# ClimateImpactLab/climate_toolbox

Hardware: AMD Instinct MI355X
Metric: gridcell-region-timesteps/sec (higher is better)
Workload: dtype f32

## Files before the change

climate_toolbox_amd/csrc/wagg_dense.hip:

```cpp
#include <algorithm>
#include <cfloat>
#include <chrono>
#include <cmath>
#include <limits>
#include <cstdlib>
#include <type_traits>

#include "wagg_dense_int.h"
#include "wagg_entry.h"

namespace wagg {

constexpr int D_MT = 23;
constexpr int D_BN = 256;
constexpr int D_ROWB = 128;
constexpr int D_THREADS = 512;
constexpr int D_WTB = D_BN * D_ROWB;
constexpr int D_WSLOTS = D_WTB / 16;
static_assert(D_WTB / 1024 == 32, "4 one-KiB W pieces per wave");
constexpr int d_xt_bytes(int mt) { return mt * 16 * D_ROWB; }
constexpr int d_buf_bytes(int mt) { return d_xt_bytes(mt) + D_WTB; }
static_assert(2 * d_buf_bytes(D_MT) <= 160 * 1024, "LDS budget");

typedef float f32x4 __attribute__((ext_vector_type(4)));
// ... 621 lines not shown
            dreg = ctx.take_input<int32_t>((size_t)n);
            dw = ctx.take_input<double>((size_t)n);
            if (!(drow || dcell) || !dreg || !dw) { set_error("build arena too small for the table"); return WAGG_ENOMEM; }
            int rc = rowptr ? copy_to_device(drow, rowptr, sizeof(int64_t) * ((size_t)G + 1), true, ctx.st)
                            : copy_to_device(dcell, cell_idx, sizeof(int32_t) * (size_t)n, true, ctx.st);
            if (rc == WAGG_OK) rc = copy_to_device(dreg, region_code, sizeof(int32_t) * (size_t)n, true, ctx.st);
            if (rc == WAGG_OK) rc = copy_to_device(dw, w_eff, sizeof(double) * (size_t)n, true, ctx.st);
            if (rc != WAGG_OK) return rc;
        }
        t_up = wall_s() - t0;
        WAGG_BUILD_STAMP(ctx, "upload");
        if (int rc = build_sorted_entries(ctx, dcell, drow, dreg, dw, n, G, R, kg, &se, general_sort)) return rc;
    }
    uint32_t *bitmap, *word_rank = nullptr;
    WAGG_TAKE(bitmap, ctx, uint32_t, n_words);
    WAGG_HIP(hipMemsetAsync(bitmap, 0, sizeof(uint32_t) * (size_t)n_words, ctx.st));
    const unsigned nblk = (unsigned)((se.n_u + 255) / 256);
    if (se.n_u > 0) {
        hipLaunchKernelGGL((table_tiles_kernel<T>), dim3(nblk), dim3(256), 0, ctx.st, (const uint64_t *)se.key.p, se.n_u, kg, n_kt, bitmap);
        WAGG_HIP(hipGetLastError());
    }
    WAGG_BUILD_STAMP(ctx, "den + tile census");
    std::vector<uint32_t> hbits, hrank;
    std::vector<int64_t> tiles;
    try {
        hbits.resize((size_t)n_words);
        hrank.resize((size_t)n_words);
        WAGG_HIP(staged_d2h(hbits.data(), bitmap, sizeof(uint32_t) * hbits.size(), ctx.st));
        int64_t cnt = 0;
        for (int64_t i = 0; i < n_words; ++i) { hrank[(size_t)i] = (uint32_t)cnt; cnt += __builtin_popcount(hbits[(size_t)i]); }
        tiles.reserve((size_t)cnt);
        for (int64_t i = 0; i < n_words; ++i)
            for (uint32_t m = hbits[(size_t)i]; m; m &= m - 1) tiles.push_back(i * 32 + __builtin_ctz(m));
    } catch (const std::bad_alloc &) { set_error("host allocation failed"); return WAGG_ENOMEM; }
    const double fill_all = (double)se.n_u / ((double)G * (double)R);
    int64_t walked = 0;
    if (se.n_u > 0) { if (int rc = spmm_list_cost(ctx, se, &walked)) return rc; }
    WAGG_BUILD_STAMP(ctx, "bitmap to host + list cost");
    const FormCost cost = table_form_cost(G, (int)sizeof(T), (int64_t)tiles.size(), n_tiles_all, walked, geo.n_rb, n_buckets, n_nt);
    bool tiled, entries;
    pick_table_form(cost, &tiled, &entries);
    if (flags == WAGG_DENSE_FORCE_FULL) { tiled = false; entries = false; }
    else if (flags == WAGG_DENSE_FORCE_TILES) { tiled = true; entries = false; }
    else if (flags == WAGG_DENSE_FORCE_ENTRIES) { tiled = false; entries = true; }
#ifdef WAGG_DIAG
    if (getenv("WAGG_DENSE_NO_TILED") && tiled) { tiled = false; entries = fill_all < SPMM_MAX_FILL; }
#else
    (void)fill_all;
#endif
    int rc = dense_alloc<T>(G, R, out, tiled ? (int64_t)tiles.size() : -1, entries);
    if (rc != WAGG_OK) return rc;
    wagg_dense *d = *out;
    WAGG_BUILD_STAMP(ctx, "plan alloc");
    auto fail = [&](int code) { (void)ctx.sync(); delete d; *out = nullptr; return code; };
    if (entries) {
        ctx.release_to(0);
        rc = spmm_build_from_sorted<T>(ctx, d, se);
        if (rc != WAGG_OK) return fail(rc);
    } else {
        hipError_t e = hipMemsetAsync(d->W.p, 0, 16 * (size_t)d->w_slots(), ctx.st);
        if (e == hipSuccess && tiled) e = dense_set_tiles(d, tiles, nullptr, ctx.st);
        if (e == hipSuccess && tiled) {
            word_rank = ctx.take<uint32_t>((size_t)n_words);
            e = word_rank ? staged_h2d(word_rank, hrank.data(), sizeof(uint32_t) * hrank.size(), ctx.st) : hipErrorOutOfMemory;
        }
        if (e == hipSuccess && se.n_u > 0) {
            hipLaunchKernelGGL((table_scatter_kernel<T>), dim3(nblk), dim3(256), 0, ctx.st, (const uint64_t *)se.key.p, (const double *)se.w.p,
                               se.n_u, kg, n_kt, (const uint32_t *)bitmap, (const uint32_t *)word_rank, reinterpret_cast<T *>(d->W.p));
            e = hipGetLastError();
        }
        if (e != hipSuccess) { set_error("densify: %s", hipGetErrorString(e)); return fail(WAGG_EHIP); }
    }
    hipError_t e = hipMemcpyAsync(d->den64.p, se.den.p, sizeof(double) * (size_t)R, hipMemcpyDeviceToDevice, ctx.st);
    if (e != hipSuccess) { set_error("densify den: %s", hipGetErrorString(e)); return fail(WAGG_EHIP); }
    rc = dense_den_to_host(d, ctx.st);
    if (rc == WAGG_OK) rc = dense_finish_scales(d, ctx.st);
    if (rc != WAGG_OK) return fail(rc);
    e = ctx.sync();
    if (e != hipSuccess) { set_error("plan build: %s", hipGetErrorString(e)); return fail(WAGG_EHIP); }
    WAGG_BUILD_STAMP(ctx, "pack + den to host");
    if (entries) d->sp.nnz = se.n_u;
    d->nnz_table = se.n_u;
    d->est_row_s[0] = cost.t_full; d->est_row_s[1] = cost.t_tiled; d->est_row_s[2] = cost.t_entries;
    d->walked_entries = walked;
    d->one_pass_sort = se.chunkwise;
    d->build.upload_s = t_up;
    d->build.total_s = wall_s() - t0;
    d->build.device_s = d->build.total_s - t_up;
    return WAGG_OK;
}

template <typename T, bool TILED, int MT, bool RM = false>
static const void *mfma_kernel_ptr() {
    if constexpr (TILED) return (const void *)dense_pieces_kernel<T, MT, RM>;
    else return (const void *)dense_mfma_kernel<T, 0, false, MT, RM>;
}
template <typename T>
static const void *pick_full_rm_kernel(int MT, bool rm) {
#define WAGG_PICK(M) case M: return rm ? (const void *)dense_mfma_kernel<T, 0, false, M, true> \
                                       : (const void *)dense_mfma_kernel<T, 256, false, M, false>
    if constexpr (sizeof(T) == 4) {
        switch (MT) { WAGG_PICK(20); WAGG_PICK(21); WAGG_PICK(22); WAGG_PICK(23); default: return nullptr; }
    } else {
        switch (MT) { WAGG_PICK(10); WAGG_PICK(11); default: return nullptr; }
    }
#undef WAGG_PICK
}

template <typename T>
static const void *pick_mfma_kernel(int MT, bool tiled, bool rm = false) {
#define WAGG_PICK(M) case M: return tiled ? (rm ? mfma_kernel_ptr<T, true, M, true>() : mfma_kernel_ptr<T, true, M>()) \
                                          : mfma_kernel_ptr<T, false, M>()
    if constexpr (sizeof(T) == 4) {
        switch (MT) {
            WAGG_PICK(1); WAGG_PICK(2); WAGG_PICK(3); WAGG_PICK(4); WAGG_PICK(5); WAGG_PICK(6); WAGG_PICK(8);
            WAGG_PICK(10); WAGG_PICK(12); WAGG_PICK(14); WAGG_PICK(16); WAGG_PICK(18); WAGG_PICK(20);
            WAGG_PICK(21); WAGG_PICK(22); WAGG_PICK(23);
            default: return nullptr;
        }
    } else {
        switch (MT) {
            WAGG_PICK(1); WAGG_PICK(2); WAGG_PICK(3); WAGG_PICK(4); WAGG_PICK(5); WAGG_PICK(6); WAGG_PICK(8);
            WAGG_PICK(10); WAGG_PICK(11);
            default: return nullptr;
        }
    }
#undef WAGG_PICK
}

static const void *pick_split_kernel(int MT) {
#define WAGG_PICK(M) case M: return (const void *)dense_split_kernel<M>
    switch (MT) {
        WAGG_PICK(1); WAGG_PICK(2); WAGG_PICK(3); WAGG_PICK(4); WAGG_PICK(5); WAGG_PICK(6); WAGG_PICK(8);
        WAGG_PICK(10); WAGG_PICK(12); WAGG_PICK(14); WAGG_PICK(16); WAGG_PICK(18); WAGG_PICK(20);
        WAGG_PICK(21); WAGG_PICK(22); WAGG_PICK(23);
        default: return nullptr;
    }
#undef WAGG_PICK
}

static int dense_apply_split(wagg_dense *d, const float *X_dev, int64_t Tn, int64_t ldx, const PackXfT<float> &xf,
                             float *out_dev, int64_t ldo, int MT, int n_mb, int S, hipStream_t st) {
    const int n_nt = d->n_nt, n_kt = d->n_kt, bm = MT * 16;
    const int kt_per_slice = (n_kt + S - 1) / S;
    const int64_t nblk = (int64_t)n_nt * n_mb * S;
    WAGG_REQUIRE(nblk < (int64_t)0x7fffffff, "grid too large");
    const void *kern = pick_split_kernel(MT);
    if (!kern) { set_error("no split kernel for MT=%d", MT); return WAGG_EINVAL; }
    const size_t need = (size_t)nblk * bm * D_BN;
    if (d->slabs.n < need) WAGG_HIP(d->slabs.alloc(need));
    const int64_t x_slots = (int64_t)n_mb * n_kt * bm * 8;
    if (d->xp.n < (size_t)x_slots * 4) WAGG_HIP(d->xp.alloc((size_t)x_slots * 4));
    if (d->xmax.n < (size_t)Tn) WAGG_HIP(d->xmax.alloc((size_t)Tn));
    const int aligned = ((ldx * sizeof(float)) % 16 == 0) && ((reinterpret_cast<uintptr_t>(X_dev) & 15) == 0) &&
                        (xf.mode != XF_EDD || (reinterpret_cast<uintptr_t>(xf.X2) & 15) == 0);
#ifdef WAGG_DIAG
    if (const char *dbg = MT == D_MT ? getenv("WAGG_SPLIT_DBG") : nullptr) {
        switch (atoi(dbg)) {
            case 1: kern = (const void *)dense_split_kernel<D_MT, 1>; break;
            case 4: kern = (const void *)dense_split_kernel<D_MT, 4>; break;
            case 5: kern = (const void *)dense_split_kernel<D_MT, 5>; break;
            case 8: kern = (const void *)dense_split_kernel<D_MT, 8>; break;
            case 9: kern = (const void *)dense_split_kernel<D_MT, 9>; break;
            default: break;
        }
    }
#endif
    const size_t shmem = 3 * (size_t)d_xt_bytes(MT);
    WAGG_HIP(allow_dynamic_lds(kern, shmem));
    unsigned *xmax = reinterpret_cast<unsigned *>(d->xmax.p);
    WAGG_HIP(hipMemsetAsync(xmax, 0, sizeof(unsigned) * (size_t)Tn, st));
    const int64_t gx = (d->G + 4095) / 4096 < 64 ? (d->G + 4095) / 4096 : 64;
    hipLaunchKernelGGL(dense_rowmax_kernel, dim3((unsigned)gx, (unsigned)Tn), dim3(256), 0, st, X_dev, ldx, d->G, xf, xmax);
    hipLaunchKernelGGL(dense_pack_x_split_kernel, dim3(256 * 16), dim3(256), 0, st, X_dev, Tn, ldx, d->G, n_kt, bm, x_slots, aligned,
                       (const unsigned *)xmax, reinterpret_cast<f16x8 *>(d->xp.p), xf, d->inf_dev);
    WAGG_HIP(hipGetLastError());
    const f16x8 *xp = reinterpret_cast<const f16x8 *>(d->xp.p);
    const float *wp = d->W.p, *wmax = d->wmax.p;
    float *slabs = d->slabs.p;
    int n_kt_a = n_kt, n_nt_a = n_nt, n_mb_a = n_mb, S_a = S, kps = kt_per_slice;
    void *args[] = {&xp, &wp, &wmax, &n_kt_a, &n_nt_a, &n_mb_a, &S_a, &kps, &slabs};
    WAGG_HIP(launch_timed_ptr(true, kern, dim3((unsigned)nblk), dim3(D_THREADS), args, shmem, st));
    hipLaunchKernelGGL(dense_reduce_split_kernel, dim3((unsigned)((d->R + 255) / 256), (unsigned)Tn), dim3(256), 0, st,
                       (const float *)slabs, n_nt, S, bm, d->R, (const float *)d->den32.p, (const unsigned *)xmax, wmax, out_dev, ldo);
    WAGG_HIP(hipGetLastError());
    return WAGG_OK;
}

template <typename T>
static int dense_apply(wagg_dense *d, const T *X_dev, int64_t Tn, int64_t ldx, const PackXfT<T> &xf,
                       T *out_dev, int64_t ldo, int ksplit, void *stream, bool exact = false) {
    typedef typename DT<T>::vec vec_t;
    WAGG_REQUIRE(d != nullptr, "dense plan is NULL");
    WAGG_REQUIRE(d->f64 == (sizeof(T) == 8), "this plan holds %s weights: use the matching wagg_dense_apply_*",
                 d->f64 ? "fp64" : "fp32");
    WAGG_REQUIRE(Tn >= 0, "T < 0");
    if (Tn == 0) return WAGG_OK;
    WAGG_REQUIRE(X_dev && out_dev, "X/out is NULL");
    WAGG_REQUIRE(xf.mode != XF_EDD || xf.X2 != nullptr, "tasmax is NULL");
    WAGG_REQUIRE(ldx >= d->G && ldo >= d->R, "ldx/ldo too small");
    WAGG_REQUIRE(ksplit >= 0 && ksplit % 8 == 0, "ksplit must be 0 or a multiple of 8");
    if (d->spmm) return spmm_apply<T>(d, X_dev, Tn, ldx, xf, out_dev, ldo, (hipStream_t)stream);
    constexpr int64_t ROWS_MAX = (int64_t)(65535 / (DT<T>::MT_MAX * 16)) * (DT<T>::MT_MAX * 16);
    if (Tn > ROWS_MAX) {
        for (int64_t t0 = 0; t0 < Tn; t0 += ROWS_MAX) {
            PackXfT<T> xg = xf;
            if (xg.X2) xg.X2 += t0 * ldx;
            const int64_t rows = Tn - t0 < ROWS_MAX ? Tn - t0 : ROWS_MAX;
            if (int rc = dense_apply<T>(d, X_dev + t0 * ldx, rows, ldx, xg, out_dev + t0 * ldo, ldo, ksplit, stream, exact)) return rc;
        }
        return WAGG_OK;
    }
    const int n_nt = d->n_nt, n_kt = d->n_kt;
    constexpr int BM_MAX = DT<T>::MT_MAX * 16;
    const int n_mb = (int)((Tn + BM_MAX - 1) / BM_MAX);
    const int rows = (int)((Tn + n_mb - 1) / n_mb);
    static const int mts32[] = {1, 2, 3, 4, 5, 6, 8, 10, 12, 14, 16, 18, 20, 21, 22, 23};
    static const int mts64[] = {1, 2, 3, 4, 5, 6, 8, 10, 11};
    int MT = DT<T>::MT_MAX;
    if constexpr (sizeof(T) == 4) { for (int m : mts32) if (m * 16 >= rows) { MT = m; break; } }
    else { for (int m : mts64) if (m * 16 >= rows) { MT = m; break; } }
    const int bm = MT * 16;
    if (n_mb >= 2) {
        const int64_t head = (int64_t)(n_mb - 1) * bm, tail = Tn - head;
        if (tail > 0) {
            int MT_tail = DT<T>::MT_MAX;
            if constexpr (sizeof(T) == 4) { for (int m : mts32) if ((int64_t)m * 16 >= tail) { MT_tail = m; break; } }
            else { for (int m : mts64) if ((int64_t)m * 16 >= tail) { MT_tail = m; break; } }
            if (MT_tail >= 4 && MT - MT_tail >= 2) {
                PackXfT<T> xt = xf;
                if (xt.X2) xt.X2 += head * ldx;
                if (int rc = dense_apply<T>(d, X_dev, head, ldx, xf, out_dev, ldo, ksplit, stream, exact)) return rc;
                return dense_apply<T>(d, X_dev + head * ldx, tail, ldx, xt, out_dev + head * ldo, ldo, ksplit, stream, exact);
            }
        }
    }
    int S = ksplit ? ksplit : pick_ksplit((int64_t)n_nt * n_mb, n_kt);
    if constexpr (sizeof(T) == 4) {
        if (!d->tiled && !exact && d->wmax.p != nullptr) return dense_apply_split(d, X_dev, Tn, ldx, xf, out_dev, ldo, MT, n_mb, S, (hipStream_t)stream);
    }
    const wagg_dense::TilePieces *tp = nullptr;
    if (d->tiled) {
        if (int rc = tile_pieces_for(d, n_mb, (hipStream_t)stream, &tp)) return rc;
        S = 1;
    }
    const int kt_per_slice = (n_kt + S - 1) / S;
    const int64_t nblk = tp ? (int64_t)tp->n_wg : (int64_t)n_nt * n_mb * S;
    WAGG_REQUIRE(nblk < (int64_t)0x7fffffff, "grid too large");
    const size_t n_slabs = tp ? (size_t)tp->n_slabs : (size_t)n_nt * n_mb * S;
    const size_t need = (n_slabs ? n_slabs : 1) * bm * D_BN * (sizeof(T) / 4);
    if (d->slabs.n < need) WAGG_HIP(d->slabs.alloc(need));
    const int64_t x_slots = (int64_t)n_mb * n_kt * bm * 8;
    if (d->xp.n < (size_t)x_slots * 4) WAGG_HIP(d->xp.alloc((size_t)x_slots * 4));
    const int aligned = ((ldx * sizeof(T)) % 16 == 0) && ((reinterpret_cast<uintptr_t>(X_dev) & 15) == 0) &&
                        (xf.mode != XF_EDD || (reinterpret_cast<uintptr_t>(xf.X2) & 15) == 0);
    const size_t shmem = 2 * (size_t)d_buf_bytes(MT);
    hipStream_t st = (hipStream_t)stream;
    const void *kern = pick_mfma_kernel<T>(MT, d->tiled);
    if (!kern) { set_error("no kernel for MT=%d", MT); return WAGG_EINVAL; }
    bool rm = xf.mode == 0 && aligned && d->G % DT<T>::BK == 0 && ((volatile int *)d->inf_host)[1] == 0;
    const void *kern_rm = nullptr;
    if (rm && d->tiled) kern_rm = pick_mfma_kernel<T>(MT, true, true);
    else if (rm && n_mb >= 2 && (kern_rm = pick_full_rm_kernel<T>(MT, true)) != nullptr) kern = pick_full_rm_kernel<T>(MT, false);
    rm = kern_rm != nullptr;
    if (rm) WAGG_HIP(allow_dynamic_lds(kern_rm, shmem));
#ifdef WAGG_DIAG
    if (getenv("WAGG_DENSE_PACKED") || (!d->tiled && getenv("WAGG_DENSE_DBG"))) {
        rm = false; kern_rm = nullptr;
        kern = pick_mfma_kernel<T>(MT, d->tiled);
    }
    if constexpr (sizeof(T) == 4) {
        if (const char *dbg = (d->tiled || MT != D_MT) ? nullptr : getenv("WAGG_DENSE_DBG")) {
            switch (atoi(dbg)) {
                case 1: kern = (const void *)dense_mfma_kernel<float, 1>; break;
                case 4: kern = (const void *)dense_mfma_kernel<float, 4>; break;
                case 5: kern = (const void *)dense_mfma_kernel<float, 5>; break;
                case 8: kern = (const void *)dense_mfma_kernel<float, 8>; break;
                case 16: kern = (const void *)dense_mfma_kernel<float, 16>; break;
                case 32: kern = (const void *)dense_mfma_kernel<float, 32>; break;
                case 64: kern = (const void *)dense_mfma_kernel<float, 64>; break;
                case 96: kern = (const void *)dense_mfma_kernel<float, 96>; break;
                case 128: kern = (const void *)dense_mfma_kernel<float, 128>; break;
                case 160: kern = (const void *)dense_mfma_kernel<float, 160>; break;
                case 192: kern = (const void *)dense_mfma_kernel<float, 192>; break;
                case 224: kern = (const void *)dense_mfma_kernel<float, 224>; break;
                default: break;
            }
        }
    }
#endif
    WAGG_HIP(allow_dynamic_lds(kern, shmem));
    const T *xp = reinterpret_cast<const T *>(d->xp.p), *wp = reinterpret_cast<const T *>(d->W.p);
    T *slabs = reinterpret_cast<T *>(d->slabs.p);
    int n_kt_a = n_kt, n_nt_a = n_nt, n_mb_a = n_mb, S_a = S, kps = kt_per_slice;
    const int32_t *tkt = d->tile_kt.p;
    const int32_t *toff = tp ? tp->tab.p : nullptr;
    const int32_t *slab_first = tp ? tp->tab.p + tp->slab_first_at : nullptr;
    int64_t ldxB = ldx * (int64_t)sizeof(T);
    int Tn_a = (int)Tn;
    const T *den;
    if constexpr (sizeof(T) == 4) den = d->den32.p; else den = d->den64.p;
    const dim3 rgrid((unsigned)((d->R + 255) / 256), (unsigned)Tn);
    const int *gate = nullptr;
    if (rm) {
        gate = d->nonfinite.p;
        WAGG_HIP(hipMemsetAsync(d->nonfinite.p, 0, sizeof(int), st));
        const int *no_gate = nullptr;
        void *args_rm[] = {&X_dev, &wp, &n_kt_a, &n_nt_a, &n_mb_a, &S_a, &kps, &slabs, &tkt, &toff, &ldxB, &Tn_a, &no_gate};
        WAGG_HIP(launch_timed_ptr(true, kern_rm, dim3((unsigned)nblk), dim3(D_THREADS), args_rm, shmem, st));
        hipLaunchKernelGGL((dense_reduce_kernel<T>), rgrid, dim3(256), 0, st, (const T *)slabs, n_nt, S, bm, Tn, d->R, den,
                           out_dev, ldo, d->nonfinite.p, (const int *)nullptr, d->inf_dev + 1, slab_first);
        WAGG_HIP(hipGetLastError());
    }
    hipLaunchKernelGGL((dense_pack_x_kernel<T>), dim3(256 * 16), dim3(256), 0, st, X_dev, Tn, ldx, d->G, n_kt, bm, x_slots,
                       aligned, reinterpret_cast<vec_t *>(d->xp.p), xf, d->inf_dev, gate);
    WAGG_HIP(hipGetLastError());
    void *args[] = {&xp, &wp, &n_kt_a, &n_nt_a, &n_mb_a, &S_a, &kps, &slabs, &tkt, &toff, &ldxB, &Tn_a, &gate};
    WAGG_HIP(launch_timed_ptr(!rm, kern, dim3((unsigned)nblk), dim3(D_THREADS), args, shmem, st));
    hipLaunchKernelGGL((dense_reduce_kernel<T>), rgrid, dim3(256), 0, st, (const T *)slabs, n_nt, S, bm, Tn, d->R, den,
                       out_dev, ldo, (int *)nullptr, gate, (int *)nullptr, slab_first);
    WAGG_HIP(hipGetLastError());
    return WAGG_OK;
}

template <typename T>
static int apply_poly(wagg_dense *d, const T *X_dev, int64_t Tn, int64_t ldx, double offset, int power, T *out_dev,
                      int64_t ldo, int ksplit, void *stream, bool exact = false) {
    WAGG_REQUIRE(power >= 1 && power <= 16, "power must lie in [1, 16], got %d", power);
// ... 282 lines not shown
```

climate_toolbox_amd/csrc/wagg_dense_int.h:

```cpp
#pragma once
#include <memory>

#include "wagg_build.h"
#include "wagg_host.h"

namespace wagg {

template <typename T> struct PackXfT {
    int mode = 0;
    T off = T(0), thr = T(0);
    const T *X2 = nullptr;
};
typedef PackXfT<float> PackXf;

template <typename T>
__device__ __forceinline__ T pack_xf(const PackXfT<T> &xf, T x, T x2, bool &inf_seen) {
    T y = x;
    if (xf.mode > 0) y = xform1<T>(x, xf.off, xf.mode);
    else if (xf.mode == XF_EDD) y = snyder_edd1<T>(x + xf.off, x2 + xf.off, xf.thr);
    inf_seen |= __builtin_isinf(y);
    return y == y ? y : T(0);
}

constexpr int SP_WAVES = 16;
constexpr int SP_THREADS = SP_WAVES * 64;
constexpr int SP_ROW = 512;
constexpr int SP_KC = 128;
constexpr int SP_ACC = 88;
constexpr int SP_RW_MAX = SP_ACC / 2 - 1;
constexpr int SP_TRASH = 2 * SP_RW_MAX;
constexpr int SP_GROUP = 8;
constexpr int SP_PAD_GROUPS = 48;
template <typename T> struct SpT {
    static constexpr int TB = SP_ROW / (int)sizeof(T);
    static constexpr int GW = 4 + 8 * (int)(sizeof(T) / 4);
    static constexpr int WSLOT = 128 * (int)sizeof(T);
};
__host__ __device__ inline unsigned sp_entry_lo(int cell_in_chunk, int j) { return (unsigned)(cell_in_chunk << 9 | 2 * j); }
template <typename T> __host__ __device__ inline int64_t sp_lo16_index(int64_t pos) {
    return (pos >> 3) * (2 * SpT<T>::GW) + (pos & 7);
}
template <typename T> __host__ __device__ inline int64_t sp_w_index(int64_t pos) {
    return (pos >> 3) * SpT<T>::GW + 4 + (pos & 7) * (int)(sizeof(T) / 4);
}

struct SpmmPlan {
    int rw = 0;
    int n_rb = 0;
    int n_chunks = 0;
    int64_t nnz = 0, n_groups = 0;
    DevBuf<uint32_t> ent;
    DevBuf<int32_t> grp_off;
};

}

struct wagg_dense {
    int64_t G = 0;
    int32_t R = 0;
    int n_kt = 0, n_nt = 0;
    bool f64 = false;
    wagg::DevBuf<float> W, den32, slabs, xp;
    wagg::DevBuf<double> den64;
    wagg::DevBuf<float> wmax, xmax;
    std::vector<double> den_host;
    bool tiled = false;
    int64_t n_tiles = 0;
    wagg::DevBuf<int32_t> tile_kt;
    std::vector<int32_t> nt_first;
    struct TilePieces {
        int n_mb = 0, n_wg = 0, n_slabs = 0;
        wagg::DevBuf<int32_t> tab;
        int64_t slab_first_at = 0;
    };
    std::vector<std::unique_ptr<TilePieces>> pieces;
    int64_t w_slots() const { return n_tiles * (8192 / 4); }
    bool spmm = false;
    wagg::SpmmPlan sp;
    int ncu = 256;
    int device = 0;
    int *inf_host = nullptr, *inf_dev = nullptr;
    wagg::DevBuf<int> nonfinite;
    int64_t nnz_table = -1;
    wagg::BuildTimes build;
    double est_row_s[3] = {0, 0, 0};
    int64_t walked_entries = 0;
    bool one_pass_sort = false;
    ~wagg_dense() { if (inf_host) wagg::note_cleanup(hipHostFree(inf_host), "hipHostFree(inf note)"); }
};

namespace wagg {
template <typename T> int spmm_build_synth(wagg_dense *d, uint32_t seed, double fill);
void spmm_geometry(int64_t G, int32_t R, SpmmPlan &sp);
template <typename T> int spmm_build_from_sorted(BuildCtx &ctx, wagg_dense *d, const SortedEntries &se);
int spmm_list_cost(BuildCtx &ctx, const SortedEntries &se, int64_t *walked_entries);
template <typename T> int spmm_apply(wagg_dense *d, const T *X, int64_t Tn, int64_t ldx, const PackXfT<T> &xf, T *out,
                                     int64_t ldo, hipStream_t stream);
int dense_alloc_common(wagg_dense *d);
}
```

climate_toolbox_amd/csrc/wagg_dense_split.inc:

```
typedef _Float16 f16x8 __attribute__((ext_vector_type(8)));

__host__ __device__ __forceinline__ int split_exp(float m) {
    int e = 0;
    if (!(m > 0.0f)) return 0;
    (void)frexpf(m, &e);
    return 15 - e;
}

typedef _Float16 f16x2 __attribute__((ext_vector_type(2)));
typedef unsigned u32x4 __attribute__((ext_vector_type(4)));
__device__ __forceinline__ void split_w8(f32x4 a, f32x4 b, int e, f16x8 &hi, f16x8 &lo) {
    u32x4 H, L;
#pragma unroll
    for (int p = 0; p < 4; ++p) {
        const float v0 = __builtin_amdgcn_ldexpf(p < 2 ? a[2 * p] : b[2 * p - 4], e);
        const float v1 = __builtin_amdgcn_ldexpf(p < 2 ? a[2 * p + 1] : b[2 * p - 3], e);
        const unsigned h = __builtin_bit_cast(unsigned, f16x2{(_Float16)v0, (_Float16)v1});
        unsigned l;
        asm("v_fma_mixlo_f16 %0, %1, -1.0, %2 op_sel_hi:[1,0,0]\n\t"
            "v_fma_mixhi_f16 %0, %1, -1.0, %3 op_sel:[1,0,0] op_sel_hi:[1,0,0]\n\t"
            "s_nop 1"
            : "=&v"(l) : "v"(h), "v"(v0), "v"(v1));
        H[p] = h;
        L[p] = l;
// ... 53 lines not shown
        const int q_ = (wave + 8 * i_) % XPIECES;                                                 \
        __builtin_amdgcn_raw_ptr_buffer_load_lds(xr, (lptr_t)(lds + (buf) * XT4 + q_ * 1024), 16, lane16, q_ * 1024, 0, 0); \
    } while (0)
#define WAGG_DMA_XALL(tile, buf)                                                                  \
    do {                                                                                          \
        const auto xr_ = WAGG_RSRC(xslice + (int64_t)(tile) * XT4, XT4);                          \
        WAGG_DMA_X(0, xr_, buf);                                                                  \
        if constexpr (NXP > 1) WAGG_DMA_X(NXP > 1 ? 1 : 0, xr_, buf);                             \
        if constexpr (NXP > 2) WAGG_DMA_X(NXP > 2 ? 2 : 0, xr_, buf);                             \
        if constexpr (NXP > 3) WAGG_DMA_X(NXP > 3 ? 3 : 0, xr_, buf);                             \
        if constexpr (NXP > 4) WAGG_DMA_X(NXP > 4 ? 4 : 0, xr_, buf);                             \
        if constexpr (NXP > 5) WAGG_DMA_X(NXP > 5 ? 5 : 0, xr_, buf);                             \
    } while (0)
#define WAGG_LOAD_W(tile)                                                                         \
    do {                                                                                          \
        const auto wr_ = WAGG_RSRC(wslice + (int64_t)(tile) * D_WTB, D_WTB);                      \
        b00 = __builtin_bit_cast(f32x4, __builtin_amdgcn_raw_buffer_load_b128(wr_, wfrag0, 0, 0));        \
        b01 = __builtin_bit_cast(f32x4, __builtin_amdgcn_raw_buffer_load_b128(wr_, wfrag1, 0, 0));        \
        b10 = __builtin_bit_cast(f32x4, __builtin_amdgcn_raw_buffer_load_b128(wr_, wfrag0 + 2048, 0, 0)); \
        b11 = __builtin_bit_cast(f32x4, __builtin_amdgcn_raw_buffer_load_b128(wr_, wfrag1 + 2048, 0, 0)); \
    } while (0)

    f32x4 acc[MT][2];
#pragma unroll
    for (int m = 0; m < MT; ++m) acc[m][0] = acc[m][1] = f32x4{0, 0, 0, 0};

    f32x4 b00, b01, b10, b11;
    if (ntiles > 0) {
        const int t1 = ntiles > 1 ? 1 : 0;
        WAGG_LOAD_W(0);
        WAGG_DMA_XALL(0, 0);
        WAGG_DMA_XALL(t1, 1);
        asm volatile("s_waitcnt vmcnt(0)" ::: "memory");
        __builtin_amdgcn_s_barrier();
    }

#define WAGG_SPLIT(A, B, E, HI, LO)                                                               \
    do {                                                                                          \
        if constexpr (DBG & 8) { HI = __builtin_bit_cast(f16x8, A); LO = __builtin_bit_cast(f16x8, B); } \
        else split_w8(A, B, E, HI, LO);                                                           \
    } while (0)
#define WAGG_MFMA16(RB, CB, A, B) acc[RB][CB] = __builtin_amdgcn_mfma_f32_16x16x32_f16(A, B, acc[RB][CB], 0, 0, 0)
#define WAGG_READ_A(H, L, RB)                                                                     \
    do {                                                                                          \
        H = *reinterpret_cast<const f16x8 *>(img + frag0 + (RB) * 2048);                          \
        L = *reinterpret_cast<const f16x8 *>(img + frag1 + (RB) * 2048);                          \
    } while (0)
    constexpr auto xdma_block = [](int i) { return MT <= 2 ? MT - 1 : 2 + i * (MT - 2) / NXP; };
#define WAGG_DMA_AT(RB, i)                                                                        \
    do {                                                                                          \
        if constexpr (!(DBG & 1) && (i) < NXP && xdma_block(i) == (RB)) WAGG_DMA_X((i) < NXP ? (i) : 0, xfar, bfar); \
    } while (0)
#define WAGG_DMA_BLOCK(RB)                                                                        \
    do {                                                                                          \
        WAGG_DMA_AT(RB, 0); WAGG_DMA_AT(RB, 1); WAGG_DMA_AT(RB, 2);                               \
        WAGG_DMA_AT(RB, 3); WAGG_DMA_AT(RB, 4); WAGG_DMA_AT(RB, 5);                               \
    } while (0)
#define WAGG_BLOCK_(RB, H, L, NH, NL)                                                             \
    do {                                                                                          \
        __builtin_amdgcn_sched_barrier(0);                                                        \
        WAGG_MFMA16(RB, 0, H, wl0);                                                               \
        __builtin_amdgcn_sched_barrier(0);                                                        \
        if constexpr ((RB) + 1 < MT) WAGG_READ_A(NH, NL, (RB) + 1 < MT ? (RB) + 1 : 0);           \
        __builtin_amdgcn_sched_barrier(0);                                                        \
        WAGG_MFMA16(RB, 1, H, wl1);                                                               \
        WAGG_MFMA16(RB, 0, L, wh0);                                                               \
        WAGG_MFMA16(RB, 1, L, wh1);                                                               \
        WAGG_MFMA16(RB, 0, H, wh0);                                                               \
        WAGG_MFMA16(RB, 1, H, wh1);                                                               \
        __builtin_amdgcn_sched_barrier(0);                                                        \
        WAGG_DMA_BLOCK(RB);                                                                       \
    } while (0)
#define WAGG_BLOCK(RB)                                                                            \
    do {                                                                                          \
        if constexpr ((RB) < MT) {                                                                \
            constexpr int rb_ = (RB) < MT ? (RB) : 0;                                             \
            if constexpr ((RB) & 1) WAGG_BLOCK_(rb_, aBh, aBl, aAh, aAl);                         \
            else WAGG_BLOCK_(rb_, aAh, aAl, aBh, aBl);                                            \
        }                                                                                         \
    } while (0)

    int bcur = 0;
    for (int tile = 0; tile < ntiles; ++tile) {
        const char *img = lds + bcur * XT4;
        const int bfar = bcur == 0 ? 2 : bcur - 1;
        const int tnext = tile + 1 < ntiles ? tile + 1 : ntiles - 1;
        const int tfar = tile + 2 < ntiles ? tile + 2 : ntiles - 1;
        const auto xfar = WAGG_RSRC(xslice + (int64_t)tfar * XT4, XT4);
        f16x8 wh0, wl0, wh1, wl1, aAh, aAl, aBh, aBl;
        WAGG_READ_A(aAh, aAl, 0);
        WAGG_SPLIT(b00, b01, ew0, wh0, wl0);
        if constexpr (MT > 1) WAGG_READ_A(aBh, aBl, MT > 1 ? 1 : 0);
        __builtin_amdgcn_sched_barrier(0);
        WAGG_MFMA16(0, 0, aAh, wl0);
        WAGG_MFMA16(0, 0, aAl, wh0);
        WAGG_MFMA16(0, 0, aAh, wh0);
        if constexpr (MT > 1) {
            WAGG_MFMA16(MT > 1 ? 1 : 0, 0, aBh, wl0);
            WAGG_MFMA16(MT > 1 ? 1 : 0, 0, aBl, wh0);
            WAGG_MFMA16(MT > 1 ? 1 : 0, 0, aBh, wh0);
        }
        WAGG_SPLIT(b10, b11, ew1, wh1, wl1);
        __builtin_amdgcn_sched_barrier(0);
        if constexpr (!(DBG & 1)) WAGG_LOAD_W(tnext);
        __builtin_amdgcn_sched_barrier(0);
        WAGG_MFMA16(0, 1, aAh, wl1);
        WAGG_MFMA16(0, 1, aAl, wh1);
        WAGG_MFMA16(0, 1, aAh, wh1);
        __builtin_amdgcn_sched_barrier(0);
        if constexpr (MT > 2) WAGG_READ_A(aAh, aAl, MT > 2 ? 2 : 0);
        __builtin_amdgcn_sched_barrier(0);
        if constexpr (MT > 1) {
            WAGG_MFMA16(MT > 1 ? 1 : 0, 1, aBh, wl1);
            WAGG_MFMA16(MT > 1 ? 1 : 0, 1, aBl, wh1);
            WAGG_MFMA16(MT > 1 ? 1 : 0, 1, aBh, wh1);
        }
        __builtin_amdgcn_sched_barrier(0);
        WAGG_DMA_BLOCK(0); WAGG_DMA_BLOCK(1);
        WAGG_BLOCK(2); WAGG_BLOCK(3); WAGG_BLOCK(4); WAGG_BLOCK(5);
        WAGG_BLOCK(6); WAGG_BLOCK(7); WAGG_BLOCK(8); WAGG_BLOCK(9); WAGG_BLOCK(10); WAGG_BLOCK(11);
        WAGG_BLOCK(12); WAGG_BLOCK(13); WAGG_BLOCK(14); WAGG_BLOCK(15); WAGG_BLOCK(16); WAGG_BLOCK(17);
        WAGG_BLOCK(18); WAGG_BLOCK(19); WAGG_BLOCK(20); WAGG_BLOCK(21); WAGG_BLOCK(22);
        static_assert(MT <= 23, "row blocks are written out up to 22");
        __builtin_amdgcn_sched_barrier(0);
        if constexpr (!(DBG & 4)) {
            __builtin_amdgcn_s_waitcnt(WAIT_TILE);
            __builtin_amdgcn_s_barrier();
        }
        bcur = bcur == 2 ? 0 : bcur + 1;
    }
    asm volatile("s_waitcnt vmcnt(0)" ::: "memory");

    float *slab = slabs + ((((int64_t)mb * n_nt + nt) * S + ks) * (MT * 16)) * D_BN;
#pragma unroll
    for (int m = 0; m < MT; ++m)
#pragma unroll
        for (int cb = 0; cb < 2; ++cb)
#pragma unroll
            for (int r = 0; r < 4; ++r)
                slab[(m * 16 + kq * 4 + r) * D_BN + wave * 32 + cb * 16 + lr] = acc[m][cb][r];
#undef WAGG_RSRC
#undef WAGG_DMA_X
#undef WAGG_DMA_XALL
#undef WAGG_LOAD_W
#undef WAGG_DMA_AT
#undef WAGG_DMA_BLOCK
#undef WAGG_SPLIT
#undef WAGG_MFMA16
#undef WAGG_READ_A
#undef WAGG_BLOCK_
#undef WAGG_BLOCK
}

__global__ void dense_rowmax_kernel(const float *__restrict__ X, int64_t ldx, int64_t G, PackXfT<float> xf,
                                    unsigned *__restrict__ rowmax) {
    const int64_t t = blockIdx.y;
    const float *src = X + t * ldx;
    const float *src2 = xf.mode == XF_EDD ? xf.X2 + t * ldx : src;
    bool inf_seen = false;
    float m = 0.0f;
    for (int64_t g = (int64_t)blockIdx.x * blockDim.x + threadIdx.x; g < G; g += (int64_t)gridDim.x * blockDim.x) {
        const float y = pack_xf<float>(xf, src[g], src2[g], inf_seen);
        const float a = fabsf(y);
        m = a <= FLT_MAX && a > m ? a : m;
    }
#pragma unroll
    for (int o = 32; o >= 1; o >>= 1) m = fmaxf(m, __shfl_xor(m, o, 64));
    __shared__ float wm[16];
    if ((threadIdx.x & 63) == 0) wm[threadIdx.x >> 6] = m;
    __syncthreads();
    if (threadIdx.x == 0) {
        for (int w = 1; w < (int)(blockDim.x >> 6); ++w) m = fmaxf(m, wm[w]);
        if (m > 0.0f) atomicMax(rowmax + t, __float_as_uint(m));
    }
}

__global__ void dense_pack_x_split_kernel(const float *__restrict__ X, int64_t Tn, int64_t ldx, int64_t G, int n_kt, int bm,
                                          int64_t n_slots, int aligned, const unsigned *__restrict__ rowmax,
                                          f16x8 *__restrict__ Xp, PackXfT<float> xf, int *__restrict__ inf_flag) {
    const int64_t stride = (int64_t)gridDim.x * blockDim.x;
    const int tile_slots = bm * 8;
    bool inf_seen = false;
    for (int64_t s = (int64_t)blockIdx.x * blockDim.x + threadIdx.x; s < n_slots; s += stride) {
        const int slot = (int)(s % tile_slots);
        const int64_t tk = s / tile_slots;
        const int kt = (int)(tk % n_kt);
        const int64_t mb = tk / n_kt;
        const int row = slot >> 3, p = (slot & 7) ^ ((row >> 1) & 7);
        const bool low = p >= 4;
        const int64_t t = mb * bm + row, k0 = (int64_t)kt * 32 + 4 * (p & 3);
        f16x8 o;
#pragma unroll
        for (int c = 0; c < 8; ++c) o[c] = (_Float16)0.0f;
        if (t < Tn) {
            const int ex = split_exp(__uint_as_float(rowmax[t]));
            const float *src = X + t * ldx;
            const float *src2 = xf.mode == XF_EDD ? xf.X2 + t * ldx : src;
            float v[8], h[8];
#pragma unroll
            for (int c = 0; c < 8; ++c) { v[c] = 0.0f; h[c] = 0.0f; }
#pragma unroll
            for (int half = 0; half < 2; ++half) {
                const int64_t kk = k0 + 16 * half;
                if (aligned && kk + 4 <= G) {
                    const f32x4 a = *reinterpret_cast<const f32x4 *>(src + kk);
                    const f32x4 b = xf.mode == XF_EDD ? *reinterpret_cast<const f32x4 *>(src2 + kk) : a;
#pragma unroll
                    for (int c = 0; c < 4; ++c) { v[4 * half + c] = a[c]; h[4 * half + c] = b[c]; }
                } else {
#pragma unroll
                    for (int c = 0; c < 4; ++c) if (kk + c < G) { v[4 * half + c] = src[kk + c]; h[4 * half + c] = src2[kk + c]; }
                }
            }
#pragma unroll
            for (int c = 0; c < 8; ++c) {
                const int64_t k = k0 + 16 * (c >> 2) + (c & 3);
                if (k >= G) continue;
                const float y = __builtin_amdgcn_ldexpf(pack_xf<float>(xf, v[c], h[c], inf_seen), ex);
                const _Float16 hi = (_Float16)y;
                o[c] = low ? (__builtin_isinf(y) ? (_Float16)0.0f : (_Float16)(y - (float)hi)) : hi;
            }
        }
        Xp[s] = o;
    }
    if (inf_seen) __hip_atomic_store(inf_flag, 1, __ATOMIC_RELAXED, __HIP_MEMORY_SCOPE_SYSTEM);
}

__global__ void dense_reduce_split_kernel(const float *__restrict__ slabs, int n_nt, int S, int bm, int32_t R,
                                          const float *__restrict__ den, const unsigned *__restrict__ rowmax,
                                          const float *__restrict__ wmax, float *__restrict__ out, int64_t ldo) {
    const int64_t r = (int64_t)blockIdx.x * blockDim.x + threadIdx.x;
    const int64_t t = blockIdx.y;
    if (r >= R) return;
    const int mb = (int)(t / bm), tl = (int)(t % bm);
    const int nt = (int)(r / D_BN), c = (int)(r % D_BN);
    const float *p = slabs + ((((int64_t)mb * n_nt + nt) * S) * bm + tl) * D_BN + c;
    float s = 0.0f;
    for (int k = 0; k < S; ++k) s += p[(int64_t)k * bm * D_BN];
    const int e = split_exp(__uint_as_float(rowmax[t])) + split_exp(wmax[r]);
    out[t * ldo + r] = __builtin_amdgcn_ldexpf(s, -e) / den[r];
}

__global__ void dense_colmax_kernel(const f32x4 *__restrict__ Wp, int n_kt, int kt_per_block, unsigned *__restrict__ wmax) {
    const int nt = blockIdx.x;
    const int ktb = blockIdx.y * kt_per_block;
    const int kte = ktb + kt_per_block < n_kt ? ktb + kt_per_block : n_kt;
    for (int slot = threadIdx.x; slot < D_WSLOTS; slot += blockDim.x) {
        float m = 0.0f;
        for (int kt = ktb; kt < kte; ++kt) {
            const f32x4 v = Wp[((int64_t)nt * n_kt + kt) * D_WSLOTS + slot];
#pragma unroll
            for (int c = 0; c < 4; ++c) { const float a = fabsf(v[c]); m = a <= FLT_MAX && a > m ? a : m; }
        }
        m = fmaxf(m, __shfl_xor(m, 1, 64));
        m = fmaxf(m, __shfl_xor(m, 2, 64));
        m = fmaxf(m, __shfl_xor(m, 4, 64));
        if ((slot & 7) == 0 && m > 0.0f) atomicMax(wmax + nt * D_BN + (slot >> 3), __float_as_uint(m));
    }
}
```

Before: 229400 billion.

## Fuse row-max into X packing using sampled scale guess and fix-up repack

Replaces the full row-max pass over X with a cheap sampled guess kernel that reads every 128th group of four elements per row. The pack kernel then scales with that guess and computes the true row max as a side effect, and a fix-up kernel repacks only rows whose exponent differs from the guess. The aim is to remove one full read of X ahead of packing. In exchange it adds a third launch and a serial dependency, and rows with outlier values outside the sampled columns pay for a second pack.

```diff
diff --git a/climate_toolbox_amd/csrc/wagg_dense.hip b/climate_toolbox_amd/csrc/wagg_dense.hip
--- a/climate_toolbox_amd/csrc/wagg_dense.hip
+++ b/climate_toolbox_amd/csrc/wagg_dense.hip
@@ -797,6 +797,7 @@
     const int64_t x_slots = (int64_t)n_mb * n_kt * bm * 8;
     if (d->xp.n < (size_t)x_slots * 4) WAGG_HIP(d->xp.alloc((size_t)x_slots * 4));
     if (d->xmax.n < (size_t)Tn) WAGG_HIP(d->xmax.alloc((size_t)Tn));
+    if (d->xguess.n < (size_t)Tn) WAGG_HIP(d->xguess.alloc((size_t)Tn));
     const int aligned = ((ldx * sizeof(float)) % 16 == 0) && ((reinterpret_cast<uintptr_t>(X_dev) & 15) == 0) &&
                         (xf.mode != XF_EDD || (reinterpret_cast<uintptr_t>(xf.X2) & 15) == 0);
 #ifdef WAGG_DIAG
@@ -815,10 +816,18 @@
     WAGG_HIP(allow_dynamic_lds(kern, shmem));
     unsigned *xmax = reinterpret_cast<unsigned *>(d->xmax.p);
     WAGG_HIP(hipMemsetAsync(xmax, 0, sizeof(unsigned) * (size_t)Tn, st));
-    const int64_t gx = (d->G + 4095) / 4096 < 64 ? (d->G + 4095) / 4096 : 64;
-    hipLaunchKernelGGL(dense_rowmax_kernel, dim3((unsigned)gx, (unsigned)Tn), dim3(256), 0, st, X_dev, ldx, d->G, xf, xmax);
-    hipLaunchKernelGGL(dense_pack_x_split_kernel, dim3(256 * 16), dim3(256), 0, st, X_dev, Tn, ldx, d->G, n_kt, bm, x_slots, aligned,
-                       (const unsigned *)xmax, reinterpret_cast<f16x8 *>(d->xp.p), xf, d->inf_dev);
+    unsigned *xguess = reinterpret_cast<unsigned *>(d->xguess.p);
+    f16x8 *xp_w = reinterpret_cast<f16x8 *>(d->xp.p);
+    hipLaunchKernelGGL(dense_rowguess_kernel, dim3((unsigned)Tn), dim3(256), 0, st, X_dev, ldx, d->G, xf, xguess);
+    const int pack_gx = std::min(n_kt, std::max(1, 4096 / n_mb));
+    const int kt_per_block = (n_kt + pack_gx - 1) / pack_gx;
+    WAGG_REQUIRE((int64_t)kt_per_block * bm * 8 < (int64_t)0x7fffffff, "k range of a pack workgroup too large");
+    hipLaunchKernelGGL(dense_pack_x_split_kernel, dim3((unsigned)((n_kt + kt_per_block - 1) / kt_per_block), (unsigned)n_mb),
+                       dim3(XPACK_THREADS), 0, st, X_dev, Tn, ldx, d->G, n_kt, bm, kt_per_block, aligned, (const unsigned *)xguess, xmax,
+                       xp_w, xf, d->inf_dev);
+    const int repack_gx = std::max(1, std::min(16, (int)(((int64_t)n_kt * 8 + XPACK_THREADS * 16 - 1) / (XPACK_THREADS * 16))));
+    hipLaunchKernelGGL(dense_repack_rows_kernel, dim3((unsigned)repack_gx, (unsigned)Tn), dim3(XPACK_THREADS), 0, st, X_dev, Tn, ldx,
+                       d->G, n_kt, bm, aligned, (const unsigned *)xguess, (const unsigned *)xmax, xp_w, xf);
     WAGG_HIP(hipGetLastError());
     const f16x8 *xp = reinterpret_cast<const f16x8 *>(d->xp.p);
     const float *wp = d->W.p, *wmax = d->wmax.p;
diff --git a/climate_toolbox_amd/csrc/wagg_dense_int.h b/climate_toolbox_amd/csrc/wagg_dense_int.h
--- a/climate_toolbox_amd/csrc/wagg_dense_int.h
+++ b/climate_toolbox_amd/csrc/wagg_dense_int.h
@@ -62,7 +62,7 @@
     bool f64 = false;
     wagg::DevBuf<float> W, den32, slabs, xp;
     wagg::DevBuf<double> den64;
-    wagg::DevBuf<float> wmax, xmax;
+    wagg::DevBuf<float> wmax, xmax, xguess;
     std::vector<double> den_host;
     bool tiled = false;
     int64_t n_tiles = 0;
diff --git a/climate_toolbox_amd/csrc/wagg_dense_split.inc b/climate_toolbox_amd/csrc/wagg_dense_split.inc
--- a/climate_toolbox_amd/csrc/wagg_dense_split.inc
+++ b/climate_toolbox_amd/csrc/wagg_dense_split.inc
@@ -229,78 +229,115 @@
 #undef WAGG_BLOCK
 }
 
-__global__ void dense_rowmax_kernel(const float *__restrict__ X, int64_t ldx, int64_t G, PackXfT<float> xf,
-                                    unsigned *__restrict__ rowmax) {
-    const int64_t t = blockIdx.y;
+
+constexpr int XG_STRIDE = 128;
+
+__global__ __launch_bounds__(256) void dense_rowguess_kernel(const float *__restrict__ X, int64_t ldx, int64_t G, PackXfT<float> xf,
+                                                             unsigned *__restrict__ xguess) {
+    const int64_t t = blockIdx.x;
     const float *src = X + t * ldx;
     const float *src2 = xf.mode == XF_EDD ? xf.X2 + t * ldx : src;
     bool inf_seen = false;
     float m = 0.0f;
-    for (int64_t g = (int64_t)blockIdx.x * blockDim.x + threadIdx.x; g < G; g += (int64_t)gridDim.x * blockDim.x) {
-        const float y = pack_xf<float>(xf, src[g], src2[g], inf_seen);
-        const float a = fabsf(y);
-        m = a <= FLT_MAX && a > m ? a : m;
+    for (int64_t g0 = (int64_t)threadIdx.x * (4 * XG_STRIDE); g0 < G; g0 += (int64_t)blockDim.x * (4 * XG_STRIDE)) {
+#pragma unroll
+        for (int c = 0; c < 4; ++c) {
+            if (g0 + c >= G) continue;
+            const float a = fabsf(pack_xf<float>(xf, src[g0 + c], src2[g0 + c], inf_seen));
+            m = a <= FLT_MAX && a > m ? a : m;
+        }
     }
 #pragma unroll
     for (int o = 32; o >= 1; o >>= 1) m = fmaxf(m, __shfl_xor(m, o, 64));
-    __shared__ float wm[16];
+    __shared__ float wm[4];
     if ((threadIdx.x & 63) == 0) wm[threadIdx.x >> 6] = m;
     __syncthreads();
-    if (threadIdx.x == 0) {
-        for (int w = 1; w < (int)(blockDim.x >> 6); ++w) m = fmaxf(m, wm[w]);
-        if (m > 0.0f) atomicMax(rowmax + t, __float_as_uint(m));
-    }
-}
-
-__global__ void dense_pack_x_split_kernel(const float *__restrict__ X, int64_t Tn, int64_t ldx, int64_t G, int n_kt, int bm,
-                                          int64_t n_slots, int aligned, const unsigned *__restrict__ rowmax,
-                                          f16x8 *__restrict__ Xp, PackXfT<float> xf, int *__restrict__ inf_flag) {
-    const int64_t stride = (int64_t)gridDim.x * blockDim.x;
+    if (threadIdx.x == 0) xguess[t] = __float_as_uint(fmaxf(fmaxf(m, wm[1]), fmaxf(wm[2], wm[3])));
+}
+
+__device__ __forceinline__ float pack_split_slot(const float *__restrict__ X, int64_t Tn, int64_t ldx, int64_t G, int n_kt, int bm,
+                                                 int aligned, const unsigned *__restrict__ rowscale, f16x8 *__restrict__ Xp,
+                                                 const PackXfT<float> &xf, int64_t mb, int kt, int row, int pos, bool &inf_seen) {
+    const int p = pos ^ ((row >> 1) & 7);
+    const bool low = p >= 4;
+    const int64_t t = mb * bm + row, k0 = (int64_t)kt * 32 + 4 * (p & 3);
+    float m = 0.0f;
+    f16x8 o;
+#pragma unroll
+    for (int c = 0; c < 8; ++c) o[c] = (_Float16)0.0f;
+    if (t < Tn) {
+        const int ex = split_exp(__uint_as_float(rowscale[t]));
+        const float *src = X + t * ldx;
+        const float *src2 = xf.mode == XF_EDD ? xf.X2 + t * ldx : src;
+        float v[8], h[8];
+#pragma unroll
+        for (int c = 0; c < 8; ++c) { v[c] = 0.0f; h[c] = 0.0f; }
+#pragma unroll
+        for (int half = 0; half < 2; ++half) {
+            const int64_t kk = k0 + 16 * half;
+            if (aligned && kk + 4 <= G) {
+                const f32x4 a = *reinterpret_cast<const f32x4 *>(src + kk);
+                const f32x4 b = xf.mode == XF_EDD ? *reinterpret_cast<const f32x4 *>(src2 + kk) : a;
+#pragma unroll
+                for (int c = 0; c < 4; ++c) { v[4 * half + c] = a[c]; h[4 * half + c] = b[c]; }
+            } else {
+#pragma unroll
+                for (int c = 0; c < 4; ++c) if (kk + c < G) { v[4 * half + c] = src[kk + c]; h[4 * half + c] = src2[kk + c]; }
+            }
+        }
+#pragma unroll
+        for (int c = 0; c < 8; ++c) {
+            const int64_t k = k0 + 16 * (c >> 2) + (c & 3);
+            if (k >= G) continue;
+            const float x = pack_xf<float>(xf, v[c], h[c], inf_seen);
+            const float a = fabsf(x);
+            m = !low && a <= FLT_MAX && a > m ? a : m;
+            const float y = __builtin_amdgcn_ldexpf(x, ex);
+            const _Float16 hi = (_Float16)y;
+            o[c] = low ? (__builtin_isinf(y) ? (_Float16)0.0f : (_Float16)(y - (float)hi)) : hi;
+        }
+    }
+    Xp[(((int64_t)mb * n_kt + kt) * bm + row) * 8 + pos] = o;
+    return m;
+}
+
+constexpr int XPACK_THREADS = 256;
+__global__ __launch_bounds__(XPACK_THREADS) void dense_pack_x_split_kernel(
+    const float *__restrict__ X, int64_t Tn, int64_t ldx, int64_t G, int n_kt, int bm, int kt_per_block, int aligned,
+    const unsigned *__restrict__ xguess, unsigned *__restrict__ rowmax, f16x8 *__restrict__ Xp, PackXfT<float> xf,
+    int *__restrict__ inf_flag) {
+    __shared__ unsigned lmax[D_MT * 16];
+    for (int r = threadIdx.x; r < bm; r += XPACK_THREADS) lmax[r] = 0u;
+    __syncthreads();
+    const int64_t mb = blockIdx.y;
+    const int kt0 = (int)blockIdx.x * kt_per_block;
+    const int kt1 = kt0 + kt_per_block < n_kt ? kt0 + kt_per_block : n_kt;
     const int tile_slots = bm * 8;
+    const int n_local = (kt1 - kt0) * tile_slots;
     bool inf_seen = false;
-    for (int64_t s = (int64_t)blockIdx.x * blockDim.x + threadIdx.x; s < n_slots; s += stride) {
-        const int slot = (int)(s % tile_slots);
-        const int64_t tk = s / tile_slots;
-        const int kt = (int)(tk % n_kt);
-        const int64_t mb = tk / n_kt;
-        const int row = slot >> 3, p = (slot & 7) ^ ((row >> 1) & 7);
-        const bool low = p >= 4;
-        const int64_t t = mb * bm + row, k0 = (int64_t)kt * 32 + 4 * (p & 3);
-        f16x8 o;
-#pragma unroll
-        for (int c = 0; c < 8; ++c) o[c] = (_Float16)0.0f;
-        if (t < Tn) {
-            const int ex = split_exp(__uint_as_float(rowmax[t]));
-            const float *src = X + t * ldx;
-            const float *src2 = xf.mode == XF_EDD ? xf.X2 + t * ldx : src;
-            float v[8], h[8];
-#pragma unroll
-            for (int c = 0; c < 8; ++c) { v[c] = 0.0f; h[c] = 0.0f; }
-#pragma unroll
-            for (int half = 0; half < 2; ++half) {
-                const int64_t kk = k0 + 16 * half;
-                if (aligned && kk + 4 <= G) {
-                    const f32x4 a = *reinterpret_cast<const f32x4 *>(src + kk);
-                    const f32x4 b = xf.mode == XF_EDD ? *reinterpret_cast<const f32x4 *>(src2 + kk) : a;
-#pragma unroll
-                    for (int c = 0; c < 4; ++c) { v[4 * half + c] = a[c]; h[4 * half + c] = b[c]; }
-                } else {
-#pragma unroll
-                    for (int c = 0; c < 4; ++c) if (kk + c < G) { v[4 * half + c] = src[kk + c]; h[4 * half + c] = src2[kk + c]; }
-                }
-            }
-#pragma unroll
-            for (int c = 0; c < 8; ++c) {
-                const int64_t k = k0 + 16 * (c >> 2) + (c & 3);
-                if (k >= G) continue;
-                const float y = __builtin_amdgcn_ldexpf(pack_xf<float>(xf, v[c], h[c], inf_seen), ex);
-                const _Float16 hi = (_Float16)y;
-                o[c] = low ? (__builtin_isinf(y) ? (_Float16)0.0f : (_Float16)(y - (float)hi)) : hi;
-            }
-        }
-        Xp[s] = o;
-    }
+    for (int li = threadIdx.x; li < n_local; li += XPACK_THREADS) {
+        const int slot = li % tile_slots, row = slot >> 3;
+        const float m = pack_split_slot(X, Tn, ldx, G, n_kt, bm, aligned, xguess, Xp, xf, mb, kt0 + li / tile_slots, row, slot & 7,
+                                        inf_seen);
+        if (m > 0.0f && __float_as_uint(m) > lmax[row]) atomicMax(&lmax[row], __float_as_uint(m));
+    }
+    __syncthreads();
+    for (int r = threadIdx.x; r < bm; r += XPACK_THREADS)
+        if (lmax[r] != 0u) atomicMax(rowmax + mb * bm + r, lmax[r]);
     if (inf_seen) __hip_atomic_store(inf_flag, 1, __ATOMIC_RELAXED, __HIP_MEMORY_SCOPE_SYSTEM);
+}
+
+__global__ __launch_bounds__(XPACK_THREADS) void dense_repack_rows_kernel(
+    const float *__restrict__ X, int64_t Tn, int64_t ldx, int64_t G, int n_kt, int bm, int aligned,
+    const unsigned *__restrict__ xguess, const unsigned *__restrict__ rowmax, f16x8 *__restrict__ Xp, PackXfT<float> xf) {
+    const int64_t t = blockIdx.y;
+    if (split_exp(__uint_as_float(rowmax[t])) == split_exp(__uint_as_float(xguess[t]))) return;
+    const int64_t mb = t / bm;
+    const int row = (int)(t % bm);
+    bool inf_seen = false;
+    const int64_t n = (int64_t)n_kt * 8;
+    for (int64_t i = (int64_t)blockIdx.x * XPACK_THREADS + threadIdx.x; i < n; i += (int64_t)gridDim.x * XPACK_THREADS)
+        (void)pack_split_slot(X, Tn, ldx, G, n_kt, bm, aligned, rowmax, Xp, xf, mb, (int)(i >> 3), row, (int)(i & 7), inf_seen);
 }
 
 __global__ void dense_reduce_split_kernel(const float *__restrict__ slabs, int n_nt, int S, int bm, int32_t R,
```

Result: no change. 231500 billion (median of 6 runs) (+0.9%).
